# DINT-NSDI24/DINT

Measured on NVIDIA H100. Metric: committed txns/sec (lock_fasst), higher is better.
Workload: dtype u32

## Files before the change

### dint_b200/csrc/engine.cu

```cuda
#include <cmath>
#include <cstdio>
#include <cstdlib>
#include <cstring>
#include <string>
#include <chrono>
#include <vector>

#include "../../include/dint_b200.h"
#include "kernels.cuh"
#include "route.cuh"
#include "kv.cuh"
#include "clients.cuh"

using namespace dint;

static thread_local std::string g_last_error;
static int set_err(int code, const char* what, cudaError_t ce = cudaSuccess) {
  char buf[512];
  if (ce != cudaSuccess) snprintf(buf, sizeof buf, "%s: %s", what, cudaGetErrorString(ce));
  else snprintf(buf, sizeof buf, "%s", what);
  g_last_error = buf;
  return code;
}
#define CU(call)                                                              \
// ... 7 lines not shown
static const uint32_t kValSize[DINT_NUM_KINDS] = {0, 0, 0, 40, 40, 8};

enum { KT_CLASSIFY = 0, KT_LOGSCAN, KT_APPLY, KT_ORDERED, KT_LOAD, KT_NUM };
static const char* kKernelNames[KT_NUM] = {"k_classify", "k_log_scan", "k_apply", "k_ordered", "k_kv_load"};

struct EvPair { cudaEvent_t a, b; int which; };
constexpr int kHostBufs = 4;

struct dint_engine {
  int kind = 0;
  int device = 0;
  dint_cfg cfg{};
  uint32_t msg = 0;
  uint32_t chunk = 0;
  uint32_t max_tiles = 0;
  bool has_log = false;
  Ctx ctx{};
  std::vector<void*> allocs;
  cudaStream_t stream = nullptr, s_in = nullptr, s_out = nullptr;
  uint8_t* d_req[kHostBufs] = {nullptr};
  uint8_t* d_resp[kHostBufs] = {nullptr};
  cudaEvent_t ev_in[kHostBufs]{}, ev_comp[kHostBufs]{}, ev_out[kHostBufs]{};
  uint32_t host_chunk = 0;
  bool plain_launches = false;
  uint32_t host_min_slice = 0;
  bool host_ramp_up = true;
  unsigned long long* h_counters = nullptr;
  unsigned long long* h_kvcnt = nullptr;
  cudaEvent_t ev_kvcnt = nullptr;
  int coop_grid = 0;
  int sms = 0;
  int grid_classify = 0, grid_apply = 0;
  uint32_t smem_stage = 0;
  uint64_t total_groups = 0;
  uint32_t* d_flags[2] = {nullptr, nullptr};
  uint32_t* d_grp[2] = {nullptr, nullptr};
  uint64_t chunk_seq = 0;
  uint32_t prev_n = 0;
  bool ord_pending = false;
  uint8_t* ord_resp = nullptr;
  const uint8_t* ord_req = nullptr;
  uint32_t ord_tile0 = 0;
  uint32_t seg_tiles = 0;
  uint64_t seg_resp[kMaxShards]{};
  bool pad_ok = false;
  const uint32_t* skip = nullptr;
  uint32_t smem_classify = 0;
  uint32_t* d_nc = nullptr;
  uint32_t* d_route = nullptr;
  uint32_t route_tiles = 0;
  uint32_t* d_route2 = nullptr;
  uint32_t route_desc_tiles = 0, route_seq = 0;
  int grid_route = 0;
  uint8_t* hot_arena = nullptr;
  size_t hot_bytes = 0;
  bool use_window = false;
  cudaAccessPolicyWindow window{};
  dint_stats stats{};
  uint32_t profiling = 0;
  std::vector<EvPair> ev_pool;
  size_t ev_used = 0;
  double kt_ms[KT_NUM] = {0};
  uint64_t kt_n[KT_NUM] = {0};
  KvHost kv[kMaxTables];
};

template <typename T>
static int dalloc(dint_engine* e, T** p, size_t count, bool zero = true) {
// ... 24 lines not shown
    e->stats.kernel_launches++;
    if (!((e->profiling >> which) & 1u)) return;
    if (e->ev_used == e->ev_pool.size()) {
      if (e->ev_pool.size() >= 8192) { prof_flush(e); }
      else {
        EvPair np{}; cudaEventCreate(&np.a); cudaEventCreate(&np.b);
        e->ev_pool.push_back(np);
      }
    }
    p = &e->ev_pool[e->ev_used++];
    p->which = which;
    cudaEventRecord(p->a, s);
  }
  ~ProfScope() { if (p) cudaEventRecord(p->b, s); }
};

template <typename... Args>
static cudaError_t launch_ex(dint_engine* e, void (*kern)(Args...), int grid, int block, size_t smem, cudaStream_t s,
                             bool coop, Args... args) {
  cudaLaunchConfig_t cfg{};
  cfg.gridDim = dim3(grid < 1 ? 1 : grid);
  cfg.blockDim = dim3(block);
  cfg.dynamicSmemBytes = smem;
  cfg.stream = s;
  cudaLaunchAttribute at[3];
  int na = 0;
  if (coop) { at[na].id = cudaLaunchAttributeCooperative; at[na].val.cooperative = 1; na++; }
  if (e->use_window) { at[na].id = cudaLaunchAttributeAccessPolicyWindow; at[na].val.accessPolicyWindow = e->window; na++; }
  cfg.attrs = at;
  cfg.numAttrs = na;
  return cudaLaunchKernelEx(&cfg, kern, args...);
}

template <int KIND, bool HAS_LOG>
static int launch_chunk_t(dint_engine* e, const Ctx& c, cudaStream_t s) {
  {
    ProfScope ps(e, s, KT_CLASSIFY);
    int want = (int)c.n_tiles, clr = (int)((c.prev_n + 4 * kTile - 1) / (4 * kTile));
    if (clr > want) want = clr;
    int grid = (want < e->grid_classify && !c.ord_pending) ? want : e->grid_classify;
    if (c.n == 0 && e->sms > 0 && grid > 8 * e->sms) grid = 8 * e->sms;
    CU(launch_ex(e, k_classify<KIND, HAS_LOG>, grid, kTile, e->smem_classify, s, false, c));
  }
  if (c.n == 0) { CU(cudaGetLastError()); return DINT_OK; }
  if (HAS_LOG) {
    ProfScope ps(e, s, KT_LOGSCAN);
    k_log_scan<<<1, kThreads, 0, s>>>(c);
  }
  {
    ProfScope ps(e, s, KT_APPLY);
    int grid = (int)c.n_tiles < e->grid_apply ? (int)c.n_tiles : e->grid_apply;
    CU(launch_ex(e, k_apply<KIND, HAS_LOG>, grid, kTile, e->smem_stage, s, false, c));
  }
  if (KIND != K_LOG) {
    ProfScope ps(e, s, KT_ORDERED);
    Ctx f = c;
    f.nc_ord = c.nc_cur;
    f.ord_resp = c.resp;
    f.ord_req = c.req;
    f.ord_tile0 = c.tile0;
    f.coop_launch = e->plain_launches ? 0u : 1u;
    int g3 = e->coop_grid;
    if (e->plain_launches && e->sms > 0) {
      const int per = g3 / e->sms;
      g3 = (per > 1 ? per - 1 : 1) * e->sms;
    }
    CU(launch_ex(e, k_ordered<KIND>, g3, kThreads, 0, s, !e->plain_launches, f));
  }
// ... 2 lines not shown
}

static int launch_chunk(dint_engine* e, const Ctx& c, cudaStream_t s) {
  switch (e->kind) {
    case DINT_LOCK2PL: return launch_chunk_t<K_LOCK2PL, false>(e, c, s);
    case DINT_FASST: return launch_chunk_t<K_FASST, false>(e, c, s);
    case DINT_LOG: return launch_chunk_t<K_LOG, true>(e, c, s);
    case DINT_STORE: return launch_chunk_t<K_STORE, false>(e, c, s);
    case DINT_TATP: return launch_chunk_t<K_TATP, true>(e, c, s);
    case DINT_SMALLBANK: return launch_chunk_t<K_SMALLBANK, true>(e, c, s);
  }
  return DINT_EINVAL;
}

template <int KIND, bool HAS_LOG>
static int grids_for(dint_engine* e) {
  int per_sm = 0, sms = 0;
  CU(cudaDeviceGetAttribute(&sms, cudaDevAttrMultiProcessorCount, e->device));
  e->sms = sms;
  e->grid_route = 4 * sms;
  e->smem_stage = Stage<Wire<KIND>::MSG>::N * Stage<Wire<KIND>::MSG>::BYTES;
  if (e->smem_stage > 48 * 1024) {
    CU(cudaFuncSetAttribute(k_classify<KIND, HAS_LOG>, cudaFuncAttributeMaxDynamicSharedMemorySize, (int)e->smem_stage));
    CU(cudaFuncSetAttribute(k_apply<KIND, HAS_LOG>, cudaFuncAttributeMaxDynamicSharedMemorySize, (int)e->smem_stage));
  }
  e->smem_classify = e->smem_stage;
  if (KIND != K_LOG && (kTile / 32) * OrdSlice<KIND>::BYTES > e->smem_classify) e->smem_classify = (kTile / 32) * OrdSlice<KIND>::BYTES;
  CU(cudaOccupancyMaxActiveBlocksPerMultiprocessor(&per_sm, k_classify<KIND, HAS_LOG>, kTile, e->smem_classify));
  if (per_sm < 1) return set_err(DINT_EIO, "k_classify cannot be resident");
  e->grid_classify = per_sm * sms;
  CU(cudaOccupancyMaxActiveBlocksPerMultiprocessor(&per_sm, k_apply<KIND, HAS_LOG>, kTile, e->smem_stage));
  if (per_sm < 1) return set_err(DINT_EIO, "k_apply cannot be resident");
  e->grid_apply = per_sm * sms;
  if (KIND == K_LOG) { e->coop_grid = 1; return DINT_OK; }
  CU(cudaOccupancyMaxActiveBlocksPerMultiprocessor(&per_sm, k_ordered<KIND>, kThreads, 0));
  if (per_sm < 1) return set_err(DINT_EIO, "k_ordered cannot be resident");
  if (per_sm > 4) per_sm = 4;
  e->coop_grid = per_sm * sms;
  return DINT_OK;
}

static void fill_chunk_ctx(dint_engine* e, Ctx& c) {
  const int cur = (int)(e->chunk_seq & 1);
  c.grp = e->d_grp[cur];
  c.grp_prev = e->d_grp[cur ^ 1];
  c.flags = e->d_flags[cur];
  c.flags_prev = e->d_flags[cur ^ 1];
  c.prev_n = e->prev_n;
  c.nc_cur = e->d_nc + 4 * cur;
  c.nc_ord = e->d_nc + 4 * (cur ^ 1);
  c.ord_pending = e->ord_pending ? 1u : 0u;
  c.ord_resp = e->ord_resp;
  c.ord_req = e->ord_req;
  c.ord_tile0 = e->ord_tile0;
  c.seg_tiles = e->seg_tiles;
  c.pad_ok = e->pad_ok ? 1u : 0u;
  c.skip = e->skip;
  for (int i = 0; i < kMaxShards; i++) c.seg_resp[i] = e->seg_resp[i];
}

static int submit_chunk(dint_engine* e, const uint8_t* req, uint32_t n, uint8_t* resp, cudaStream_t s, uint32_t tile0 = 0) {
  Ctx c = e->ctx;
  c.n = n;
  c.n_tiles = (n + kTile - 1) / kTile;
  c.req = req;
  c.resp = resp;
  c.tile0 = tile0;
  fill_chunk_ctx(e, c);
  int rc = launch_chunk(e, c, s);
  if (rc) return rc;
  e->chunk_seq++;
  e->prev_n = n;
  e->ord_pending = e->kind != DINT_LOG;
  e->ord_resp = resp;
  e->ord_req = req;
  e->ord_tile0 = tile0;
  e->stats.chunks++;
  e->stats.requests += n;
  return DINT_OK;
}

static int flush_ordered(dint_engine* e, cudaStream_t s) {
  if (!e->ord_pending) return DINT_OK;
  Ctx c = e->ctx;
  c.n = 0;
  c.n_tiles = 0;
  c.req = nullptr;
  c.resp = nullptr;
  fill_chunk_ctx(e, c);
  c.prev_n = 0;
  int rc = launch_chunk(e, c, s);
  if (rc) return rc;
  e->ord_pending = false;
  return DINT_OK;
}

static int kv_maintain(dint_engine* e, cudaStream_t s) {
  if (e->ctx.n_tables == 0) return DINT_OK;
  if (!e->h_kvcnt) {
    CU(cudaHostAlloc((void**)&e->h_kvcnt, 2 * kMaxTables * sizeof(unsigned long long), cudaHostAllocDefault));
    memset(e->h_kvcnt, 0, 2 * kMaxTables * sizeof(unsigned long long));
    CU(cudaEventCreateWithFlags(&e->ev_kvcnt, cudaEventDisableTiming));
    return DINT_OK;
  }
  if (cudaEventQuery(e->ev_kvcnt) != cudaSuccess) { cudaGetLastError(); return DINT_OK; }
  for (uint32_t t = 0; t < e->ctx.n_tables; t++) {
// ... 211 lines not shown
  c.shard_id = cf.shard_id;
  c.shard_div = make_fastmod(cf.n_shards);
  c.slot_mod = make_fastmod(cf.lock_slots);
  c.ring_n = cf.log_ring ? cf.log_ring : 1;

  uint64_t groups = 0;
  auto local_groups = [&](uint64_t global) { return (global + cf.n_shards - 1) / cf.n_shards; };
  int rc;
  switch (e->kind) {
    case DINT_LOCK2PL:
      groups = local_groups(cf.lock_slots);
      if ((rc = dalloc(e, &c.cnt2, groups))) return rc;
      break;
    case DINT_FASST:
      groups = local_groups(cf.lock_slots);
      if ((rc = dalloc(e, &c.ver, groups))) return rc;
      break;
    case DINT_LOG:
      groups = 0;
      break;
    default:
      if ((rc = kv_create_tables(e->kind, cf, c, e->kv, &groups,
                                 [&](void** p, size_t bytes) -> int {
                                   uint8_t* q = nullptr;
                                   int r = dalloc(e, &q, bytes);
                                   *p = q;
                                   return r;
                                 })))
        return rc == DINT_EINVAL ? set_err(rc, "bad KV configuration") : rc;
      break;
  }
  e->total_groups = groups;
  if (groups >= 0xffffffffULL) return set_err(DINT_EINVAL, "too many groups");
  {
    uint32_t fl = 25;
    while (fl > 10 && (1ULL << (fl - 1)) >= groups * 2 + 2048) fl--;
    c.flags_mask = (1u << fl) - 1;
    const size_t set_bytes = (size_t)4 << (fl - 3);
    const size_t lock_bytes = (e->kind == DINT_FASST) ? (((groups + 31) / 32) * 4 + 255) / 256 * 256 : 0;
    e->hot_bytes = 2 * set_bytes + lock_bytes;
    if ((rc = dalloc(e, &e->hot_arena, e->hot_bytes))) return rc;
    e->d_flags[0] = (uint32_t*)e->hot_arena;
    e->d_flags[1] = (uint32_t*)(e->hot_arena + set_bytes);
    if (lock_bytes) c.lockbits = (uint32_t*)(e->hot_arena + 2 * set_bytes);
    int max_persist = 0, max_win = 0;
    cudaDeviceGetAttribute(&max_persist, cudaDevAttrMaxPersistingL2CacheSize, e->device);
    cudaDeviceGetAttribute(&max_win, cudaDevAttrMaxAccessPolicyWindowSize, e->device);
    if (max_persist > 0 && max_win > 0) {
      size_t want = e->hot_bytes < (size_t)max_persist ? e->hot_bytes : (size_t)max_persist;
      if (cudaDeviceSetLimit(cudaLimitPersistingL2CacheSize, want) == cudaSuccess) {
        e->window.base_ptr = e->hot_arena;
        e->window.num_bytes = e->hot_bytes < (size_t)max_win ? e->hot_bytes : (size_t)max_win;
        e->window.hitRatio = (float)((double)want / (double)e->window.num_bytes > 1.0 ? 1.0 : (double)want / (double)e->window.num_bytes);
        e->window.hitProp = cudaAccessPropertyPersisting;
        e->window.missProp = cudaAccessPropertyStreaming;
        e->use_window = true;
      } else cudaGetLastError();
    }
  }
  uint32_t bits = 1;
  while ((1ULL << bits) < groups) bits++;
  c.sort_passes = (bits + 7) / 8;

  if (e->has_log) {
    if ((rc = dalloc(e, &c.ring, (size_t)c.ring_n * kLogEntry[e->kind]))) return rc;
  }
  const uint32_t ch = e->chunk;
  e->max_tiles = (ch + kTile - 1) / kTile;
  for (int i = 0; i < 2; i++)
    if ((rc = dalloc(e, &e->d_grp[i], ch))) return rc;
  if ((rc = dalloc(e, &c.clist, (size_t)e->max_tiles * kTile))) return rc;
  if ((rc = dalloc(e, &c.ccnt, e->max_tiles))) return rc;
  if ((rc = dalloc(e, &c.cprefix, e->max_tiles + 1))) return rc;
  if ((rc = dalloc(e, &e->d_nc, 8))) return rc;
  {
    uint32_t lg = 0;
    while (((uint64_t)kBucketFill << lg) < ch) lg++;
    c.bucket_log2 = lg;
    if ((rc = dalloc(e, &c.buckets, ((size_t)1 << lg) * kBucketCap, false))) return rc;
    if ((rc = dalloc(e, &c.bcnt, (size_t)1 << lg))) return rc;
  }
  if ((rc = dalloc(e, &c.sortA, ch))) return rc;
  if ((rc = dalloc(e, &c.sortB, ch))) return rc;
  if ((rc = dalloc(e, &c.ghist, (size_t)256 * ((ch + kSortTile - 1) / kSortTile)))) return rc;
  if ((rc = dalloc(e, &c.rowtot, 256))) return rc;
  if ((rc = dalloc(e, &c.log_tilecnt, e->max_tiles))) return rc;
  if ((rc = dalloc(e, &c.log_tilebase, e->max_tiles))) return rc;
  if ((rc = dalloc(e, &c.log_total, 2))) return rc;
  if ((rc = dalloc(e, &c.counters, 4))) return rc;
  if ((rc = dalloc(e, &c.gbar, 4))) return rc;

  switch (e->kind) {
    case DINT_LOCK2PL: rc = grids_for<K_LOCK2PL, false>(e); break;
    case DINT_FASST: rc = grids_for<K_FASST, false>(e); break;
    case DINT_LOG: rc = grids_for<K_LOG, true>(e); break;
    case DINT_STORE: rc = grids_for<K_STORE, false>(e); break;
    case DINT_TATP: rc = grids_for<K_TATP, true>(e); break;
    default: rc = grids_for<K_SMALLBANK, true>(e); break;
  }
  if (rc) return rc;
  int coop = 0;
  CU(cudaDeviceGetAttribute(&coop, cudaDevAttrCooperativeLaunch, e->device));
  if (!coop) return set_err(DINT_ENODEV, "device lacks cooperative launch");
  CU(cudaStreamSynchronize(e->stream));
  return DINT_OK;
}

int dint_create(int kind, const dint_cfg* cfg, int device, dint_engine** out) {
  if (!out || kind < 0 || kind >= DINT_NUM_KINDS) return set_err(DINT_EINVAL, "bad kind/out");
  *out = nullptr;
  int ndev = 0;
  cudaError_t ce = cudaGetDeviceCount(&ndev);
  if (ce != cudaSuccess || ndev == 0) {
    cudaGetLastError();
    return set_err(DINT_ENODEV, "no CUDA device: dint_b200 has no CPU fallback");
  }
  if (device < 0 || device >= ndev) return set_err(DINT_EINVAL, "bad device ordinal");
  dint_engine* e = new dint_engine();
  e->kind = kind;
  e->device = device;
  if (cfg) e->cfg = *cfg; else dint_default_cfg(kind, &e->cfg);
  dint_cfg& cf = e->cfg;
  if (cf.n_shards == 0) cf.n_shards = 1;
  if (cf.shard_id >= cf.n_shards || cf.lock_slots == 0) { delete e; return set_err(DINT_EINVAL, "bad shard/lock_slots"); }
  if (cf.chunk == 0) cf.chunk = 1u << 20;
  e->chunk = (cf.chunk + kTile - 1) / kTile * kTile;
  {
    const uint32_t want = 1u << 18;
    e->host_chunk = want < e->chunk ? want : e->chunk;
    e->host_min_slice = 131072u;
    e->host_ramp_up = true;
  }
  e->msg = kMsgSize[kind];
// ... 167 lines not shown
  unsigned long long before = e->stats.errors;
  if ((rc = pull_counters(e))) return rc;
  return e->stats.errors != before ? DINT_EPROTO : DINT_OK;
}

int dint_submit_device(dint_engine* e, const void* req_dev, uint64_t n, void* resp_dev, void* cuda_stream) {
  if (!e || (n && (!req_dev || !resp_dev))) return set_err(DINT_EINVAL, "null argument");
  if (((uintptr_t)req_dev | (uintptr_t)resp_dev) & 15) return set_err(DINT_EINVAL, "device buffers must be 16-byte aligned");
  CU(cudaSetDevice(e->device));
  cudaStream_t s = (cudaStream_t)cuda_stream;
  return run_device(e, (const uint8_t*)req_dev, n, (uint8_t*)resp_dev, s);
}

int dint_submit(dint_engine* e, const void* req, uint64_t n, void* resp) {
  if (!e || (n && (!req || !resp))) return set_err(DINT_EINVAL, "null argument");
  CU(cudaSetDevice(e->device));
  const uint32_t hchunk = e->host_chunk;
  if (!e->d_req[0]) {
    for (int i = 0; i < kHostBufs; i++) {
      int rc;
      if ((rc = dalloc(e, &e->d_req[i], (size_t)hchunk * e->msg + 16, false))) return rc;
      if ((rc = dalloc(e, &e->d_resp[i], (size_t)hchunk * e->msg + 16, false))) return rc;
    }
  }
  static const bool trace = getenv("DINT_HOST_TRACE") != nullptr;
  const auto t_begin = std::chrono::steady_clock::now();
  CU(cudaDeviceSynchronize());
  { int rc = kv_maintain(e, e->stream); if (rc) return rc; }
  const uint8_t* rq = (const uint8_t*)req;
  uint8_t* rs = (uint8_t*)resp;
  unsigned long long err_before = e->stats.errors;
  uint64_t k = 0;
  uint64_t prev_off = 0, prev_bytes = 0;
  auto copy_out_prev = [&](uint64_t kk) -> int {
    int pb = (int)((kk - 1) % kHostBufs);
    CU(cudaEventRecord(e->ev_comp[pb], e->stream));
    CU(cudaStreamWaitEvent(e->s_out, e->ev_comp[pb], 0));
    CU(cudaMemcpyAsync(rs + prev_off, e->d_resp[pb], prev_bytes, cudaMemcpyDeviceToHost, e->s_out));
    CU(cudaEventRecord(e->ev_out[pb], e->s_out));
    return DINT_OK;
  };
  HostSlices sched(n, e->host_min_slice, hchunk, e->host_ramp_up);
  uint64_t off = 0;
  for (uint64_t cn; (cn = sched.next()) != 0; k++) {
    int b = (int)(k % kHostBufs);
    size_t bytes = (size_t)cn * e->msg;
    if (k >= (uint64_t)kHostBufs) CU(cudaStreamWaitEvent(e->s_in, e->ev_comp[b], 0));
    CU(cudaMemcpyAsync(e->d_req[b], rq + off * e->msg, bytes, cudaMemcpyHostToDevice, e->s_in));
    CU(cudaEventRecord(e->ev_in[b], e->s_in));
    CU(cudaStreamWaitEvent(e->stream, e->ev_in[b], 0));
    if (k >= (uint64_t)kHostBufs) CU(cudaStreamWaitEvent(e->stream, e->ev_out[b], 0));
    int rc = submit_chunk(e, e->d_req[b], (uint32_t)cn, e->d_resp[b], e->stream);
    if (rc) return rc;
    if (k >= 1 && (rc = copy_out_prev(k))) return rc;
    prev_off = off * e->msg;
    prev_bytes = bytes;
    e->stats.h2d_bytes += bytes;
    e->stats.d2h_bytes += bytes;
    off += cn;
  }
  {
    int rc = flush_ordered(e, e->stream);
    if (rc) return rc;
    if (k >= 1 && (rc = copy_out_prev(k))) return rc;
  }
  if (!e->h_counters) CU(cudaHostAlloc((void**)&e->h_counters, 4 * sizeof(unsigned long long), cudaHostAllocDefault));
  CU(cudaMemcpyAsync(e->h_counters, e->ctx.counters, 4 * sizeof(unsigned long long), cudaMemcpyDeviceToHost, e->stream));
  { int rc2 = kv_publish_counts(e, e->stream); if (rc2) return rc2; }
  const auto t_enq = std::chrono::steady_clock::now();
  CU(cudaStreamSynchronize(e->s_out));
  CU(cudaStreamSynchronize(e->stream));
  int rc = prof_flush(e);
  if (rc) return rc;
  if (trace) {
    const auto t_end = std::chrono::steady_clock::now();
    fprintf(stderr, "[dint_submit] n=%llu slices=%llu enqueue=%.1f us total=%.1f us\n", (unsigned long long)n, (unsigned long long)k,
            std::chrono::duration<double, std::micro>(t_enq - t_begin).count(),
            std::chrono::duration<double, std::micro>(t_end - t_begin).count());
  }
  e->stats.errors = e->h_counters[0];
  e->stats.conflicted = e->h_counters[1];
  e->stats.max_run = e->h_counters[2];
  return e->stats.errors != err_before ? DINT_EPROTO : DINT_OK;
}

struct dint_snapshot {
  dint_engine* e = nullptr;
  std::vector<std::pair<void*, size_t>> live;
  std::vector<void*> copy;
  uint64_t kv_cap[kMaxTables]{};
};
static void snapshot_regions(dint_engine* e, std::vector<std::pair<void*, size_t>>& r) {
  const Ctx& c = e->ctx;
  const uint64_t g = e->total_groups;
  if (e->kind == DINT_LOCK2PL || e->kind == DINT_SMALLBANK) r.push_back({c.cnt2, g * sizeof(uint2)});
  if (e->kind == DINT_FASST) { r.push_back({c.ver, g * sizeof(uint32_t)}); r.push_back({c.lockbits, ((g + 31) / 32) * 4}); }
  if (e->kind == DINT_TATP) r.push_back({c.lockbits, ((g + 31) / 32) * 4});
// ... 475 lines not shown
  if (c->flags) cudaFree(c->flags);
  if (c->side) cudaStreamDestroy(c->side);
  if (c->ret) cudaStreamDestroy(c->ret);
  if (c->s_in) cudaStreamDestroy(c->s_in);
  if (c->s_out) cudaStreamDestroy(c->s_out);
  c->e->plain_launches = false;
  delete c;
}

int dint_shard_flags(dint_shard_ctx* c, uint32_t out[2]) {
  if (!c || !out) return DINT_EINVAL;
  CU(cudaSetDevice(c->e->device));
  CU(cudaDeviceSynchronize());
  CU(cudaMemcpy(out, c->flags, 2 * sizeof(uint32_t), cudaMemcpyDeviceToHost));
  CU(cudaMemset(c->flags, 0, 2 * sizeof(uint32_t)));
  return DINT_OK;
}

int dint_shard_recover(dint_shard_ctx* c, uint32_t k_last, uint32_t* first_unserved) {
  if (!c || !first_unserved) return DINT_EINVAL;
  dint_engine* e = c->e;
  CU(cudaSetDevice(e->device));
  CU(cudaDeviceSynchronize());
  uint32_t bad = 0;
  CU(cudaMemcpy(&bad, c->flags + 2, sizeof bad, cudaMemcpyDeviceToHost));
  *first_unserved = 0xffffffffu;
  if (!bad) return DINT_OK;
  const uint32_t first_epoch = c->epoch - k_last + 1;
  *first_unserved = bad >= first_epoch ? bad - first_epoch : 0;
  CU(cudaMemset(c->flags, 0, 4 * sizeof(uint32_t)));
  e->ord_pending = false;
  e->prev_n = 0;
  CU(cudaMemset(e->d_nc, 0, 8 * sizeof(uint32_t)));
  CU(cudaMemset(e->d_flags[0], 0, (size_t)((char*)e->d_flags[1] - (char*)e->d_flags[0]) * 2));
  CU(cudaDeviceSynchronize());
  return DINT_OK;
}

int dint_shard_submit_many(dint_shard_ctx* c, uint32_t k, const void* const* req_dev, const uint8_t* const* dst_dev, uint64_t n,
                           void* const* out_dev, void* cuda_stream) {
  if (!c || !req_dev || !out_dev || n == 0 || n > c->max_n) return set_err(DINT_EINVAL, "bad argument");
  if (k == 0) return DINT_OK;
  std::vector<std::vector<ShardBatch>> b(1, std::vector<ShardBatch>(k));
  for (uint32_t j = 0; j < k; j++) b[0][j] = ShardBatch{req_dev[j], dst_dev ? dst_dev[j] : nullptr, out_dev[j], n};
  cudaStream_t main = (cudaStream_t)cuda_stream;
  return shard_run(&c, 1, k, b, &main);
}

}

extern "C" {

int dint_shard_submit_many_v(dint_shard_ctx* c, uint32_t k, const void* const* req_dev, const uint8_t* const* dst_dev, const uint64_t* n,
                             const uint32_t* cap, void* const* out_dev, void* cuda_stream) {
  if (!c || !req_dev || !out_dev || !n) return set_err(DINT_EINVAL, "bad argument");
  if (k == 0) return DINT_OK;
  std::vector<std::vector<ShardBatch>> b(1, std::vector<ShardBatch>(k));
  for (uint32_t j = 0; j < k; j++) {
    const uint32_t cj = cap ? cap[j] : 0;
    if (n[j] > c->max_n || cj > c->cap || cj % kTile != 0) return set_err(DINT_EINVAL, "batch size / slab capacity (a multiple of 128, <= the capacity of dint_shard_create)");
    b[0][j] = ShardBatch{req_dev[j], dst_dev ? dst_dev[j] : nullptr, out_dev[j], n[j], cj};
  }
  cudaStream_t main = (cudaStream_t)cuda_stream;
  return shard_run(&c, 1, k, b, &main);
}

int dint_shard_submit_host(dint_shard_ctx* c, uint32_t k, const void* const* req_host, const uint8_t* const* dst_host, uint64_t n,
// ... 284 lines not shown
```

### dint_b200/csrc/kernels.cuh

```cuda
#pragma once
#include <cooperative_groups.h>
#include "engine.cuh"

namespace dint {
namespace cg = cooperative_groups;

DINT_D uint32_t lane_id() { return threadIdx.x & 31; }
DINT_D uint32_t warp_id() { return threadIdx.x >> 5; }

DINT_D uint32_t tile_rank(bool flag, uint32_t* scratch, uint32_t& total) {
  uint32_t bal = __ballot_sync(0xffffffffu, flag);
  uint32_t in_warp = __popc(bal & ((1u << lane_id()) - 1u));
  if (lane_id() == 0) scratch[warp_id()] = __popc(bal);
  __syncthreads();
  uint32_t off = 0, tot = 0;
#pragma unroll
  for (int w = 0; w < kTile / 32; w++) {
    uint32_t v = scratch[w];
    if (w < (int)warp_id()) off += v;
    tot += v;
  }
  __syncthreads();
  total = tot;
  return off + in_warp;
// ... 4 lines not shown
  const uint32_t lt = (1u << lane_id()) - 1u;
  if (lane_id() == 0) scratch[warp_id()] = __popc(ba) | (__popc(bb) << 16);
  __syncthreads();
  uint32_t off = 0, tot = 0;
#pragma unroll
  for (int w = 0; w < kTile / 32; w++) {
    uint32_t v = scratch[w];
    if (w < (int)warp_id()) off += v;
    tot += v;
  }
  ra = (off & 0xffffu) + __popc(ba & lt);
  rb = (off >> 16) + __popc(bb & lt);
  ta = tot & 0xffffu;
  tb = tot >> 16;
}

DINT_D uint32_t bucket_of(uint32_t g, uint32_t log2p) { return log2p ? (g * 0x9E3779B1u) >> (32 - log2p) : 0; }

template <int MSG> struct Stage {
  static constexpr uint32_t BYTES = ((kTile * MSG + 16 + 127) / 128) * 128;
  static constexpr uint32_t N = (BYTES > 8192) ? 2 : kStages;
};

struct TileIter {
  uint32_t n_my;
  DINT_D uint32_t tile(uint32_t i) const { return blockIdx.x + i * gridDim.x; }
  DINT_D bool has(uint32_t i) const { return i < n_my; }
};
DINT_D TileIter tile_iter(uint32_t n_tiles) {
  TileIter it;
  it.n_my = blockIdx.x < n_tiles ? (n_tiles - blockIdx.x + gridDim.x - 1) / gridDim.x : 0;
  return it;
}
template <int MSG>
DINT_D void issue_tile_load(const Ctx& c, uint8_t* smem, uint64_t* full, const TileIter& it, uint32_t i) {
  const uint32_t t = it.tile(i), first = t * kTile;
  const uint32_t cnt = min((uint32_t)kTile, c.n - first);
  const uint32_t body = (cnt * MSG) & ~15u;
  const uint32_t buf = i % Stage<MSG>::N;
  if (body) {
    mbar_expect_tx(&full[buf], body);
    tma_load_1d(smem + buf * Stage<MSG>::BYTES, c.req + (size_t)first * MSG, body, &full[buf]);
  }
}
template <int MSG>
DINT_D uint8_t* acquire_tile(const Ctx& c, uint8_t* smem, uint64_t* full, const TileIter& it, uint32_t i,
                             uint32_t& first, uint32_t& cnt) {
  const uint32_t t = it.tile(i);
  first = t * kTile;
  cnt = min((uint32_t)kTile, c.n - first);
  const uint32_t bytes = cnt * MSG, body = bytes & ~15u;
  uint8_t* tile = smem + (i % Stage<MSG>::N) * Stage<MSG>::BYTES;
  if (body) mbar_wait(&full[i % Stage<MSG>::N], (i / Stage<MSG>::N) & 1u);
  if (body != bytes) {
    const uint8_t* src = c.req + (size_t)first * MSG;
    for (uint32_t b = body + threadIdx.x; b < bytes; b += blockDim.x) tile[b] = src[b];
    __syncthreads();
  }
  return tile;
}

template <int KIND>
DINT_D uint32_t route_owner_of(const Ctx& c, const uint8_t* rec) {
  using W = Wire<KIND>;
  const TypeInfo ti = type_info<KIND>(rec);
  if (ti.invalid || !ti.mask) return c.shard_id;
  uint32_t gglobal = 0;
  if constexpr (KIND == K_LOCK2PL || KIND == K_FASST) gglobal = fast_mod(fasthash64_u32(ld_u32_unaligned(rec + W::KEY)), c.slot_mod);
  else if constexpr (KIND == K_STORE) gglobal = fast_mod(fasthash64_u64(ld_u64_unaligned(rec + W::KEY)), c.tbl[0].lock_mod);
  else if constexpr (KIND == K_TATP || KIND == K_SMALLBANK) gglobal = fast_mod(fasthash64_u64(ld_u64_unaligned(rec + W::KEY)), c.tbl[rec[W::TABLE]].lock_mod);
  else return c.shard_id;
  return gglobal - (uint32_t)fast_div(gglobal, c.shard_div) * c.n_shards;
}
template <int KIND>
__global__ void __launch_bounds__(kThreads) k_route_owner(const Ctx c, const uint8_t* req, uint32_t n, uint8_t* owner) {
  const uint32_t i = blockIdx.x * kThreads + threadIdx.x;
  if (i < n) owner[i] = (uint8_t)route_owner_of<KIND>(c, req + (size_t)i * Wire<KIND>::MSG);
}

constexpr int kMaxShards = 8;
__global__ void __launch_bounds__(kThreads) k_exact_count(const uint8_t* owner, uint32_t n, uint32_t world, uint32_t* tilecnt) {
  __shared__ uint32_t cnt[kMaxShards];
  if (threadIdx.x < kMaxShards) cnt[threadIdx.x] = 0;
  __syncthreads();
  const uint32_t i = blockIdx.x * kThreads + threadIdx.x;
  const uint32_t o = i < n ? owner[i] : 0xffu;
// ... 60 lines not shown
    __threadfence_system();
    volatile uint32_t* flag = (volatile uint32_t*)sig.p[threadIdx.x] + me;
    asm volatile("st.release.sys.global.u32 [%0], %1;" ::"l"(flag), "r"(epoch) : "memory");
  }
}
constexpr uint32_t kSigOverflow = 0x80000000u;
__global__ void k_p2p_wait(const uint32_t* my_sig, uint32_t world, uint32_t epoch, uint32_t* timeout, uint32_t* bad) {
  if (threadIdx.x < world) {
    const long long t0 = clock64();
    uint32_t v;
    do {
      asm volatile("ld.acquire.sys.global.u32 %0, [%1];" : "=r"(v) : "l"(my_sig + threadIdx.x) : "memory");
      if (clock64() - t0 > 8000000000LL) { atomicExch(timeout, 1u); break; }
    } while ((int32_t)((v & ~kSigOverflow) - epoch) < 0);
    if (bad && (v & kSigOverflow) && (v & ~kSigOverflow) == epoch) atomicCAS(bad, 0u, epoch);
  }
  __syncthreads();
  __threadfence_system();
}

template <int MSG>
__global__ void __launch_bounds__(kThreads) k_exact_unpermute(const uint8_t* sorted, const uint32_t* perm, uint32_t n, uint8_t* out) {
  const uint32_t pos = blockIdx.x * kThreads + threadIdx.x;
  if (pos >= n) return;
  const uint32_t idx = perm[pos];
  if (idx == 0xffffffffu) return;
  copy_record<MSG>(out + (size_t)idx * MSG, sorted + (size_t)pos * MSG);
}

template <int KIND> struct OrdSlice {
  static constexpr uint32_t BYTES = kBucketCap * (FastReplay<KIND>::ok ? (8 + 8 + 4) : 8);
};
template <int KIND> DINT_D void ordered_buckets(const Ctx& c, uint8_t* scratch);

template <int KIND, bool HAS_LOG>
__global__ void __launch_bounds__(kTile) k_classify(const Ctx c) {
  using W = Wire<KIND>;
  constexpr uint32_t NS = Stage<W::MSG>::N;
  extern __shared__ __align__(128) uint8_t smem[];
  __shared__ uint64_t full[kStages];
  __shared__ uint32_t scratch[kTile / 32];
  if (c.skip && __ldcg(c.skip)) return;
  if (threadIdx.x == 0) {
    for (int s = 0; s < kStages; s++) mbar_init(&full[s], 1);
    if (blockIdx.x == 0) { c.nc_cur[0] = 0; c.nc_cur[1] = 0; c.nc_ord[2] = 0; }
  }
  __syncthreads();
  const bool do_ord = c.ord_pending && c.nc_ord[0] != 0 && c.nc_ord[1] == 0;
  const bool ord_first = (blockIdx.x & 1u) != 0;
  if (do_ord && ord_first) {
    ordered_buckets<KIND>(c, smem);
    __syncthreads();
  }
  const TileIter it = tile_iter(c.n_tiles);
  if (threadIdx.x == 0)
    for (uint32_t i = 0; i < NS && i < it.n_my; i++) issue_tile_load<W::MSG>(c, smem, full, it, i);

  for (uint32_t i = blockIdx.x * kTile + threadIdx.x; i < c.prev_n; i += 4 * gridDim.x * kTile) {
    uint32_t g[4];
#pragma unroll
    for (int u = 0; u < 4; u++) {
      const uint32_t j = i + u * gridDim.x * kTile;
      g[u] = j < c.prev_n ? __ldcg(&c.grp_prev[j]) : kNoGroup;
    }
#pragma unroll
    for (int u = 0; u < 4; u++)
      if (g[u] != kNoGroup) c.flags_prev[flag_word(c, g[u])] = 0;
  }

  uint32_t pend_old = 0, pend_test = 0, pend_sh = 0;
  uint32_t* pend_w = nullptr;
  bool saw_writer = false;
  for (uint32_t i = 0; it.has(i); i++) {
    if (threadIdx.x == 0 && i && i + NS - 1 < it.n_my) issue_tile_load<W::MSG>(c, smem, full, it, i + NS - 1);
    uint32_t first, cnt;
    const uint8_t* tile = acquire_tile<W::MSG>(c, smem, full, it, i, first, cnt);
    const bool valid = threadIdx.x < cnt;
    bool is_log = false;
    uint32_t new_old = 0, new_test = 0, new_sh = 0;
    uint32_t* new_w = nullptr;
    if (valid) {
      const uint8_t* rec = tile + threadIdx.x * W::MSG;
      TypeInfo ti = (c.pad_ok && rec[W::TYPE] == kPadType) ? TypeInfo{0, false, false} : type_info<KIND>(rec);
      uint32_t g = kNoGroup;
      if (!ti.invalid && ti.mask) {
        g = key_info<KIND>(c, rec).grp;
        if (g != kNoGroup) {
          uint32_t* w = &c.flags[flag_word(c, g)];
          const uint32_t sh = flag_shift(g);
          if (ti.mask == C_RA) {
            atomicOr(w, F_R << sh);
          } else {
            const uint32_t bits = ((ti.mask & C_RA) ? F_R : 0u) | ((ti.mask & C_WA) ? F_WA : 0u) | ((ti.mask & C_WL) ? F_WL : 0u);
            saw_writer = true;
            new_old = atomicOr(w, bits << sh);
            new_test = ((ti.mask & C_WA) ? F_WA : 0u) | ((ti.mask & C_WL) ? F_WL : 0u);
            new_w = w;
            new_sh = sh;
          }
        }
      }
      c.grp[first + threadIdx.x] = g;
      is_log = !ti.invalid && ti.is_log;
    }
    if (pend_w && ((pend_old >> pend_sh) & pend_test)) atomicOr(pend_w, F_W2 << pend_sh);
    pend_old = new_old; pend_test = new_test; pend_sh = new_sh; pend_w = new_w;
    if (HAS_LOG) {
      uint32_t total;
      (void)tile_rank(is_log, scratch, total);
      if (threadIdx.x == 0) c.log_tilecnt[it.tile(i)] = total;
    } else {
      __syncthreads();
    }
  }
  if (pend_w && ((pend_old >> pend_sh) & pend_test)) atomicOr(pend_w, F_W2 << pend_sh);
  if (__syncthreads_or(saw_writer ? 1 : 0) && threadIdx.x == 0) atomicOr(&c.nc_cur[2], 1u);
  if (do_ord && !ord_first) {
    __syncthreads();
    ordered_buckets<KIND>(c, smem);
  }
}

__global__ void __launch_bounds__(kThreads) k_log_scan(const Ctx c) {
  if (c.skip && __ldcg(c.skip)) return;
  __shared__ unsigned long long carry;
  __shared__ uint32_t wsum[kThreads / 32];
  if (threadIdx.x == 0) carry = c.log_total[0];
  __syncthreads();
  for (uint32_t base = 0; base < c.n_tiles; base += kThreads) {
// ... 44 lines not shown
  for (uint32_t i = 0; it.has(i); i++) {
    uint32_t* scratch = scratch2[i & 1];
    uint32_t g_k1 = kNoGroup;
    if (kGrpFromK1) {
      const uint32_t idx = it.tile(i) * kTile + threadIdx.x;
      if (idx < c.n) g_k1 = __ldcg(&c.grp[idx]);
    }
    if (threadIdx.x == 0 && i && i + NS - 1 < it.n_my) {
      asm volatile("cp.async.bulk.wait_group.read 0;" ::: "memory");
      issue_tile_load<W::MSG>(c, smem, full, it, i + NS - 1);
    }
    uint32_t first, cnt;
    uint8_t* tile = acquire_tile<W::MSG>(c, smem, full, it, i, first, cnt);
    const uint32_t t = it.tile(i);
    const bool valid = threadIdx.x < cnt;
    uint8_t* rec = tile + threadIdx.x * W::MSG;
    TypeInfo ti{0, false, false};
    KeyInfo ki{0, 0, kNoGroup};
    Pre<KIND> pf;
    bool listed = false;
    const bool pad = valid && c.pad_ok && rec[W::TYPE] == kPadType;
    if (valid && !pad) {
      ti = type_info<KIND>(rec);
      if (!ti.invalid && ti.mask) {
        if (kGrpFromK1) ki.grp = g_k1; else ki = key_info<KIND>(c, rec);
        if (ki.grp == kNoGroup) ti.invalid = true;
      }
    }
    {
      const bool active = valid && !ti.invalid && ti.mask;
      pf = prefetch_coop<KIND>(c, rec, ki, ti, active);
      if (active && chunk_has_writer) {
        const uint32_t f = (__ldcg(&c.flags[flag_word(c, ki.grp)]) >> flag_shift(ki.grp)) & 15u;
        listed = ((ti.mask & C_RA) && (f & F_WA)) || ((ti.mask & C_WA) && (f & (F_R | F_W2))) ||
                 ((ti.mask & C_WL) && (f & F_W2));
      }
    }
    unsigned long long log_ord = 0;
    bool log_keep = false;
    {
      const bool lg = HAS_LOG && valid && !ti.invalid && ti.is_log;
      uint32_t r_list, r_log, n_list, n_log;
      tile_rank2(listed, lg, scratch, r_list, r_log, n_list, n_log);
      if (lg) {
        log_ord = c.log_tilebase[t] + r_log;
        log_keep = log_ord + c.ring_n >= c.log_total[1];
      }
      if (listed) {
        const uint32_t idx = first + threadIdx.x;
        c.clist[(size_t)t * kTile + r_list] = idx;
        const uint32_t b = bucket_of(ki.grp, c.bucket_log2);
        const uint32_t pos = atomicAdd(&c.bcnt[b], 1u);
        if (pos < kBucketCap) c.buckets[(size_t)b * kBucketCap + pos] = ((uint64_t)ki.grp << 32) | idx;
        else atomicAdd(&c.nc_cur[1], 1u);
      }
      if (threadIdx.x == 0) {
        c.ccnt[t] = n_list;
        if (n_list) atomicAdd(&c.nc_cur[0], n_list);
      }
    }
    if (valid && !pad) {
      if (ti.invalid) mark_invalid<KIND>(c, rec);
      else if (!listed) apply_one<KIND>(c, rec, ki, pf, log_ord, log_keep);
    }
    const uint32_t bytes = cnt * W::MSG, body = bytes & ~15u;
    uint8_t* gdst = c.seg_tiles ? seg_tile_ptr<W::MSG>(c, c.tile0 + t) : c.resp + (size_t)first * W::MSG;
    fence_proxy_async_smem();
    __syncthreads();
    for (uint32_t b = body + threadIdx.x; b < bytes; b += blockDim.x) gdst[b] = tile[b];
    if (threadIdx.x == 0) {
      if (body) tma_store_1d(gdst, tile, body);
      asm volatile("cp.async.bulk.commit_group;" ::: "memory");
    }
  }
  if (threadIdx.x == 0) asm volatile("cp.async.bulk.wait_group 0;" ::: "memory");
}

constexpr int kSortItems = 8;
constexpr int kSortTile = kThreads * kSortItems;

template <int KIND>
DINT_D void replay_run(const Ctx& c, const uint64_t* sorted, uint32_t p, uint32_t nc) {
  using W = Wire<KIND>;
  const uint32_t g = (uint32_t)(sorted[p] >> 32);
  uint32_t len = 0;
  for (uint32_t q = p; q < nc; q++) {
    uint64_t e = sorted[q];
    if ((uint32_t)(e >> 32) != g) break;
    __align__(4) uint8_t rec[(W::MSG + 3) / 4 * 4];
    copy_record<W::MSG>(rec, c.ord_req + (size_t)(uint32_t)e * W::MSG);
    const TypeInfo ti = type_info<KIND>(rec);
    const KeyInfo ki = key_info<KIND>(c, rec);
    const Pre<KIND> pf = prefetch<KIND>(c, rec, ki, ti);
    apply_one<KIND>(c, rec, ki, pf, 0, false);
    copy_record<W::MSG>(ord_out_ptr<W::MSG>(c, (uint32_t)e), rec);
    len++;
  }
  if (len > 1) atomicMax(&c.counters[2], (unsigned long long)len);
}

template <int KIND>
DINT_D void ordered_buckets(const Ctx& c, uint8_t* scratch) {
    uint64_t* wkeys = (uint64_t*)(scratch + (size_t)warp_id() * OrdSlice<KIND>::BYTES);
    uint64_t* wres = wkeys + kBucketCap;
    uint32_t* wops = (uint32_t*)(wkeys + 2 * kBucketCap);
    const uint32_t lane = lane_id();
    const uint32_t warps_per_cta = blockDim.x / 32;
    const uint32_t n_warps = gridDim.x * warps_per_cta;
// ... 440 lines not shown
```

Before: 280.5 million.

## Fuse classify, apply and ordered replay into one cooperative kernel for FASST/2PL

Result: faster. 380.0 million (median of 6 runs) (+35.5%).

```diff
diff --git a/dint_b200/csrc/engine.cu b/dint_b200/csrc/engine.cu
--- a/dint_b200/csrc/engine.cu
+++ b/dint_b200/csrc/engine.cu
@@ -63,8 +63,11 @@
   int sms = 0;
   int grid_classify = 0, grid_apply = 0;
   uint32_t smem_stage = 0;
+  bool fused_kind = false;
+  int grid_fused = 0;
   uint64_t total_groups = 0;
   uint32_t* d_flags[2] = {nullptr, nullptr};
+  size_t flag_set_bytes = 0;
   uint32_t* d_grp[2] = {nullptr, nullptr};
   uint64_t chunk_seq = 0;
   uint32_t prev_n = 0;
@@ -155,8 +158,32 @@
   return cudaLaunchKernelEx(&cfg, kern, args...);
 }
 
+static bool fused_path(const dint_engine* e) { return e->fused_kind && !e->plain_launches; }
+
 template <int KIND, bool HAS_LOG>
 static int launch_chunk_t(dint_engine* e, const Ctx& c, cudaStream_t s) {
+  if constexpr (KIND == K_FASST || KIND == K_LOCK2PL) {
+    if (fused_path(e)) {
+      Ctx f = c;
+      f.flags = e->d_flags[0];
+      f.nc_ord = c.nc_cur;
+      f.ord_resp = c.resp;
+      f.ord_req = c.req;
+      f.ord_tile0 = c.tile0;
+      f.coop_launch = 1;
+      {
+        ProfScope ps(e, s, KT_APPLY);
+        const int grid = (int)c.n_tiles < e->grid_fused ? (int)c.n_tiles : e->grid_fused;
+        CU(launch_ex(e, k_fused<KIND>, grid, kTile, Fused<KIND>::SMEM, s, true, f));
+      }
+      {
+        ProfScope ps(e, s, KT_ORDERED);
+        CU(launch_ex(e, k_ordered<KIND>, e->coop_grid, kThreads, 0, s, true, f));
+      }
+      CU(cudaGetLastError());
+      return DINT_OK;
+    }
+  }
   {
     ProfScope ps(e, s, KT_CLASSIFY);
     int want = (int)c.n_tiles, clr = (int)((c.prev_n + 4 * kTile - 1) / (4 * kTile));
@@ -225,6 +252,12 @@
   CU(cudaOccupancyMaxActiveBlocksPerMultiprocessor(&per_sm, k_apply<KIND, HAS_LOG>, kTile, e->smem_stage));
   if (per_sm < 1) return set_err(DINT_EIO, "k_apply cannot be resident");
   e->grid_apply = per_sm * sms;
+  if constexpr (KIND == K_FASST || KIND == K_LOCK2PL) {
+    CU(cudaOccupancyMaxActiveBlocksPerMultiprocessor(&per_sm, k_fused<KIND>, kTile, Fused<KIND>::SMEM));
+    if (per_sm < 1) return set_err(DINT_EIO, "k_fused cannot be resident");
+    e->fused_kind = true;
+    e->grid_fused = per_sm * sms;
+  }
   if (KIND == K_LOG) { e->coop_grid = 1; return DINT_OK; }
   CU(cudaOccupancyMaxActiveBlocksPerMultiprocessor(&per_sm, k_ordered<KIND>, kThreads, 0));
   if (per_sm < 1) return set_err(DINT_EIO, "k_ordered cannot be resident");
@@ -259,12 +292,17 @@
   c.req = req;
   c.resp = resp;
   c.tile0 = tile0;
+  const bool fused = fused_path(e);
+  if (fused && e->prev_n) {
+    CU(cudaMemsetAsync(e->d_flags[(e->chunk_seq - 1) & 1], 0, e->flag_set_bytes, s));
+    e->prev_n = 0;
+  }
   fill_chunk_ctx(e, c);
   int rc = launch_chunk(e, c, s);
   if (rc) return rc;
   e->chunk_seq++;
-  e->prev_n = n;
-  e->ord_pending = e->kind != DINT_LOG;
+  e->prev_n = fused ? 0 : n;
+  e->ord_pending = !fused && e->kind != DINT_LOG;
   e->ord_resp = resp;
   e->ord_req = req;
   e->ord_tile0 = tile0;
@@ -542,17 +580,37 @@
   }
   e->total_groups = groups;
   if (groups >= 0xffffffffULL) return set_err(DINT_EINVAL, "too many groups");
+  switch (e->kind) {
+    case DINT_LOCK2PL: rc = grids_for<K_LOCK2PL, false>(e); break;
+    case DINT_FASST: rc = grids_for<K_FASST, false>(e); break;
+    case DINT_LOG: rc = grids_for<K_LOG, true>(e); break;
+    case DINT_STORE: rc = grids_for<K_STORE, false>(e); break;
+    case DINT_TATP: rc = grids_for<K_TATP, true>(e); break;
+    default: rc = grids_for<K_SMALLBANK, true>(e); break;
+  }
+  if (rc) return rc;
+  if (e->fused_kind) {
+    const uint64_t cap = (uint64_t)e->grid_fused * kFuseTiles * kTile;
+    if (e->chunk > cap) e->chunk = (uint32_t)cap;
+    if (e->host_chunk > e->chunk) e->host_chunk = e->chunk;
+  }
   {
     uint32_t fl = 25;
     while (fl > 10 && (1ULL << (fl - 1)) >= groups * 2 + 2048) fl--;
     c.flags_mask = (1u << fl) - 1;
     const size_t set_bytes = (size_t)4 << (fl - 3);
+    e->flag_set_bytes = set_bytes;
     const size_t lock_bytes = (e->kind == DINT_FASST) ? (((groups + 31) / 32) * 4 + 255) / 256 * 256 : 0;
-    e->hot_bytes = 2 * set_bytes + lock_bytes;
+    const size_t hot_sets = e->fused_kind ? 1 : 2;
+    e->hot_bytes = hot_sets * set_bytes + lock_bytes;
     if ((rc = dalloc(e, &e->hot_arena, e->hot_bytes))) return rc;
     e->d_flags[0] = (uint32_t*)e->hot_arena;
-    e->d_flags[1] = (uint32_t*)(e->hot_arena + set_bytes);
-    if (lock_bytes) c.lockbits = (uint32_t*)(e->hot_arena + 2 * set_bytes);
+    if (e->fused_kind) {
+      if ((rc = dalloc(e, &e->d_flags[1], set_bytes / 4))) return rc;
+    } else {
+      e->d_flags[1] = (uint32_t*)(e->hot_arena + set_bytes);
+    }
+    if (lock_bytes) c.lockbits = (uint32_t*)(e->hot_arena + hot_sets * set_bytes);
     int max_persist = 0, max_win = 0;
     cudaDeviceGetAttribute(&max_persist, cudaDevAttrMaxPersistingL2CacheSize, e->device);
     cudaDeviceGetAttribute(&max_win, cudaDevAttrMaxAccessPolicyWindowSize, e->device);
@@ -600,15 +658,6 @@
   if ((rc = dalloc(e, &c.counters, 4))) return rc;
   if ((rc = dalloc(e, &c.gbar, 4))) return rc;
 
-  switch (e->kind) {
-    case DINT_LOCK2PL: rc = grids_for<K_LOCK2PL, false>(e); break;
-    case DINT_FASST: rc = grids_for<K_FASST, false>(e); break;
-    case DINT_LOG: rc = grids_for<K_LOG, true>(e); break;
-    case DINT_STORE: rc = grids_for<K_STORE, false>(e); break;
-    case DINT_TATP: rc = grids_for<K_TATP, true>(e); break;
-    default: rc = grids_for<K_SMALLBANK, true>(e); break;
-  }
-  if (rc) return rc;
   int coop = 0;
   CU(cudaDeviceGetAttribute(&coop, cudaDevAttrCooperativeLaunch, e->device));
   if (!coop) return set_err(DINT_ENODEV, "device lacks cooperative launch");
@@ -842,11 +891,12 @@
   unsigned long long err_before = e->stats.errors;
   uint64_t k = 0;
   uint64_t prev_off = 0, prev_bytes = 0;
-  auto copy_out_prev = [&](uint64_t kk) -> int {
-    int pb = (int)((kk - 1) % kHostBufs);
+  bool pending = false;
+  auto copy_out = [&](uint64_t kk, uint64_t at, uint64_t nbytes) -> int {
+    int pb = (int)(kk % kHostBufs);
     CU(cudaEventRecord(e->ev_comp[pb], e->stream));
     CU(cudaStreamWaitEvent(e->s_out, e->ev_comp[pb], 0));
-    CU(cudaMemcpyAsync(rs + prev_off, e->d_resp[pb], prev_bytes, cudaMemcpyDeviceToHost, e->s_out));
+    CU(cudaMemcpyAsync(rs + at, e->d_resp[pb], nbytes, cudaMemcpyDeviceToHost, e->s_out));
     CU(cudaEventRecord(e->ev_out[pb], e->s_out));
     return DINT_OK;
   };
@@ -862,7 +912,9 @@
     if (k >= (uint64_t)kHostBufs) CU(cudaStreamWaitEvent(e->stream, e->ev_out[b], 0));
     int rc = submit_chunk(e, e->d_req[b], (uint32_t)cn, e->d_resp[b], e->stream);
     if (rc) return rc;
-    if (k >= 1 && (rc = copy_out_prev(k))) return rc;
+    if (pending && (rc = copy_out(k - 1, prev_off, prev_bytes))) return rc;
+    pending = e->ord_pending;
+    if (!pending && (rc = copy_out(k, off * e->msg, bytes))) return rc;
     prev_off = off * e->msg;
     prev_bytes = bytes;
     e->stats.h2d_bytes += bytes;
@@ -872,7 +924,7 @@
   {
     int rc = flush_ordered(e, e->stream);
     if (rc) return rc;
-    if (k >= 1 && (rc = copy_out_prev(k))) return rc;
+    if (pending && (rc = copy_out(k - 1, prev_off, prev_bytes))) return rc;
   }
   if (!e->h_counters) CU(cudaHostAlloc((void**)&e->h_counters, 4 * sizeof(unsigned long long), cudaHostAllocDefault));
   CU(cudaMemcpyAsync(e->h_counters, e->ctx.counters, 4 * sizeof(unsigned long long), cudaMemcpyDeviceToHost, e->stream));
@@ -1414,7 +1466,8 @@
   e->ord_pending = false;
   e->prev_n = 0;
   CU(cudaMemset(e->d_nc, 0, 8 * sizeof(uint32_t)));
-  CU(cudaMemset(e->d_flags[0], 0, (size_t)((char*)e->d_flags[1] - (char*)e->d_flags[0]) * 2));
+  CU(cudaMemset(e->d_flags[0], 0, e->flag_set_bytes));
+  CU(cudaMemset(e->d_flags[1], 0, e->flag_set_bytes));
   CU(cudaDeviceSynchronize());
   return DINT_OK;
 }
diff --git a/dint_b200/csrc/kernels.cuh b/dint_b200/csrc/kernels.cuh
--- a/dint_b200/csrc/kernels.cuh
+++ b/dint_b200/csrc/kernels.cuh
@@ -60,26 +60,26 @@
   it.n_my = blockIdx.x < n_tiles ? (n_tiles - blockIdx.x + gridDim.x - 1) / gridDim.x : 0;
   return it;
 }
-template <int MSG>
+template <int MSG, uint32_t NB = Stage<MSG>::N, uint32_t BUF = Stage<MSG>::BYTES>
 DINT_D void issue_tile_load(const Ctx& c, uint8_t* smem, uint64_t* full, const TileIter& it, uint32_t i) {
   const uint32_t t = it.tile(i), first = t * kTile;
   const uint32_t cnt = min((uint32_t)kTile, c.n - first);
   const uint32_t body = (cnt * MSG) & ~15u;
-  const uint32_t buf = i % Stage<MSG>::N;
+  const uint32_t buf = i % NB;
   if (body) {
     mbar_expect_tx(&full[buf], body);
-    tma_load_1d(smem + buf * Stage<MSG>::BYTES, c.req + (size_t)first * MSG, body, &full[buf]);
-  }
-}
-template <int MSG>
+    tma_load_1d(smem + buf * BUF, c.req + (size_t)first * MSG, body, &full[buf]);
+  }
+}
+template <int MSG, uint32_t NB = Stage<MSG>::N, uint32_t BUF = Stage<MSG>::BYTES>
 DINT_D uint8_t* acquire_tile(const Ctx& c, uint8_t* smem, uint64_t* full, const TileIter& it, uint32_t i,
                              uint32_t& first, uint32_t& cnt) {
   const uint32_t t = it.tile(i);
   first = t * kTile;
   cnt = min((uint32_t)kTile, c.n - first);
   const uint32_t bytes = cnt * MSG, body = bytes & ~15u;
-  uint8_t* tile = smem + (i % Stage<MSG>::N) * Stage<MSG>::BYTES;
-  if (body) mbar_wait(&full[i % Stage<MSG>::N], (i / Stage<MSG>::N) & 1u);
+  uint8_t* tile = smem + (i % NB) * BUF;
+  if (body) mbar_wait(&full[i % NB], (i / NB) & 1u);
   if (body != bytes) {
     const uint8_t* src = c.req + (size_t)first * MSG;
     for (uint32_t b = body + threadIdx.x; b < bytes; b += blockDim.x) tile[b] = src[b];
@@ -206,6 +206,28 @@
   static constexpr uint32_t BYTES = kBucketCap * (FastReplay<KIND>::ok ? (8 + 8 + 4) : 8);
 };
 template <int KIND> DINT_D void ordered_buckets(const Ctx& c, uint8_t* scratch);
+
+DINT_D uint32_t flag_bits(uint32_t mask) {
+  return ((mask & C_RA) ? F_R : 0u) | ((mask & C_WA) ? F_WA : 0u) | ((mask & C_WL) ? F_WL : 0u);
+}
+DINT_D uint32_t writer_bits(uint32_t mask) { return ((mask & C_WA) ? F_WA : 0u) | ((mask & C_WL) ? F_WL : 0u); }
+DINT_D bool conflicts(uint32_t mask, uint32_t f) {
+  return ((mask & C_RA) && (f & F_WA)) || ((mask & C_WA) && (f & (F_R | F_W2))) || ((mask & C_WL) && (f & F_W2));
+}
+DINT_D void list_request(const Ctx& c, uint32_t t, uint32_t first, bool listed, uint32_t grp, uint32_t r_list, uint32_t n_list) {
+  if (listed) {
+    const uint32_t idx = first + threadIdx.x;
+    c.clist[(size_t)t * kTile + r_list] = idx;
+    const uint32_t b = bucket_of(grp, c.bucket_log2);
+    const uint32_t pos = atomicAdd(&c.bcnt[b], 1u);
+    if (pos < kBucketCap) c.buckets[(size_t)b * kBucketCap + pos] = ((uint64_t)grp << 32) | idx;
+    else atomicAdd(&c.nc_cur[1], 1u);
+  }
+  if (threadIdx.x == 0) {
+    c.ccnt[t] = n_list;
+    if (n_list) atomicAdd(&c.nc_cur[0], n_list);
+  }
+}
 
 template <int KIND, bool HAS_LOG>
 __global__ void __launch_bounds__(kTile) k_classify(const Ctx c) {
@@ -265,10 +287,9 @@
           if (ti.mask == C_RA) {
             atomicOr(w, F_R << sh);
           } else {
-            const uint32_t bits = ((ti.mask & C_RA) ? F_R : 0u) | ((ti.mask & C_WA) ? F_WA : 0u) | ((ti.mask & C_WL) ? F_WL : 0u);
             saw_writer = true;
-            new_old = atomicOr(w, bits << sh);
-            new_test = ((ti.mask & C_WA) ? F_WA : 0u) | ((ti.mask & C_WL) ? F_WL : 0u);
+            new_old = atomicOr(w, flag_bits(ti.mask) << sh);
+            new_test = writer_bits(ti.mask);
             new_w = w;
             new_sh = sh;
           }
@@ -379,8 +400,7 @@
       pf = prefetch_coop<KIND>(c, rec, ki, ti, active);
       if (active && chunk_has_writer) {
         const uint32_t f = (__ldcg(&c.flags[flag_word(c, ki.grp)]) >> flag_shift(ki.grp)) & 15u;
-        listed = ((ti.mask & C_RA) && (f & F_WA)) || ((ti.mask & C_WA) && (f & (F_R | F_W2))) ||
-                 ((ti.mask & C_WL) && (f & F_W2));
+        listed = conflicts(ti.mask, f);
       }
     }
     unsigned long long log_ord = 0;
@@ -393,18 +413,7 @@
         log_ord = c.log_tilebase[t] + r_log;
         log_keep = log_ord + c.ring_n >= c.log_total[1];
       }
-      if (listed) {
-        const uint32_t idx = first + threadIdx.x;
-        c.clist[(size_t)t * kTile + r_list] = idx;
-        const uint32_t b = bucket_of(ki.grp, c.bucket_log2);
-        const uint32_t pos = atomicAdd(&c.bcnt[b], 1u);
-        if (pos < kBucketCap) c.buckets[(size_t)b * kBucketCap + pos] = ((uint64_t)ki.grp << 32) | idx;
-        else atomicAdd(&c.nc_cur[1], 1u);
-      }
-      if (threadIdx.x == 0) {
-        c.ccnt[t] = n_list;
-        if (n_list) atomicAdd(&c.nc_cur[0], n_list);
-      }
+      list_request(c, t, first, listed, ki.grp, r_list, n_list);
     }
     if (valid && !pad) {
       if (ti.invalid) mark_invalid<KIND>(c, rec);
@@ -421,6 +430,134 @@
     }
   }
   if (threadIdx.x == 0) asm volatile("cp.async.bulk.wait_group 0;" ::: "memory");
+}
+
+constexpr int kFuseTiles = 8;
+template <int KIND> struct Fused {
+  static constexpr uint32_t TILE = (kTile * Wire<KIND>::MSG + 15) / 16 * 16;
+  static constexpr uint32_t TILES = kFuseTiles * TILE;
+  static constexpr uint32_t REPLAY = (kTile / 32) * OrdSlice<KIND>::BYTES;
+  static constexpr uint32_t GRP = TILES > REPLAY ? TILES : REPLAY;
+  static constexpr uint32_t SMEM = GRP + kFuseTiles * kTile * 4;
+};
+
+template <int KIND>
+__global__ void __launch_bounds__(kTile, 8) k_fused(const Ctx c) {
+  using W = Wire<KIND>;
+  using F = Fused<KIND>;
+  extern __shared__ __align__(128) uint8_t smem[];
+  __shared__ uint64_t full[kFuseTiles];
+  __shared__ uint32_t scratch2[2][kTile / 32];
+  uint32_t* s_grp = (uint32_t*)(smem + F::GRP);
+  cg::grid_group grid = cg::this_grid();
+  const TileIter it = tile_iter(c.n_tiles);
+  const uint32_t tid = threadIdx.x;
+  if (tid == 0) {
+    for (int s = 0; s < kFuseTiles; s++) mbar_init(&full[s], 1);
+    if (blockIdx.x == 0) { c.nc_cur[0] = 0; c.nc_cur[1] = 0; }
+  }
+  __syncthreads();
+  if (tid == 0)
+    for (uint32_t i = 0; i < it.n_my; i++) issue_tile_load<W::MSG, kFuseTiles, F::TILE>(c, smem, full, it, i);
+
+  Pre<KIND> pf[kFuseTiles];
+  uint32_t old[kFuseTiles];
+  uint32_t wtest = 0;
+  bool saw_writer = false;
+#pragma unroll
+  for (int i = 0; i < kFuseTiles; i++) {
+    old[i] = 0;
+    pf[i] = Pre<KIND>{};
+    if (!it.has(i)) continue;
+    uint32_t first, cnt;
+    const uint8_t* tile = acquire_tile<W::MSG, kFuseTiles, F::TILE>(c, smem, full, it, i, first, cnt);
+    uint32_t g = kNoGroup;
+    if (tid < cnt) {
+      const uint8_t* rec = tile + tid * W::MSG;
+      const TypeInfo ti = type_info<KIND>(rec);
+      if (!ti.invalid) {
+        const KeyInfo ki = key_info<KIND>(c, rec);
+        g = ki.grp;
+        if (g != kNoGroup) {
+          uint32_t* w = &c.flags[flag_word(c, g)];
+          const uint32_t sh = flag_shift(g);
+          if (ti.mask == C_RA) {
+            atomicOr(w, F_R << sh);
+          } else {
+            saw_writer = true;
+            old[i] = atomicOr(w, flag_bits(ti.mask) << sh);
+            wtest |= writer_bits(ti.mask) << (4 * i);
+          }
+          pf[i] = prefetch<KIND>(c, rec, ki, ti);
+        }
+      }
+      c.grp[first + tid] = g;
+    }
+    s_grp[i * kTile + tid] = g;
+  }
+#pragma unroll
+  for (int i = 0; i < kFuseTiles; i++) {
+    const uint32_t test = (wtest >> (4 * i)) & 15u;
+    if (test) {
+      const uint32_t g = s_grp[i * kTile + tid];
+      if ((old[i] >> flag_shift(g)) & test) atomicOr(&c.flags[flag_word(c, g)], F_W2 << flag_shift(g));
+    }
+  }
+  if (__syncthreads_or(saw_writer ? 1 : 0) && tid == 0) atomicOr(&c.nc_cur[2], 1u);
+  grid.sync();
+
+  const bool chunk_has_writer = __ldcg(&c.nc_cur[2]) != 0;
+  uint32_t fl[kFuseTiles];
+#pragma unroll
+  for (int i = 0; i < kFuseTiles; i++) {
+    fl[i] = 0;
+    const uint32_t g = it.has(i) ? s_grp[i * kTile + tid] : kNoGroup;
+    if (chunk_has_writer && g != kNoGroup) fl[i] = (__ldcg(&c.flags[flag_word(c, g)]) >> flag_shift(g)) & 15u;
+  }
+#pragma unroll
+  for (int i = 0; i < kFuseTiles; i++) {
+    if (!it.has(i)) continue;
+    const uint32_t t = it.tile(i), first = t * kTile, cnt = min((uint32_t)kTile, c.n - first);
+    uint8_t* rec = smem + i * F::TILE + tid * W::MSG;
+    const bool valid = tid < cnt;
+    const uint32_t g = s_grp[i * kTile + tid];
+    const TypeInfo ti = valid ? type_info<KIND>(rec) : TypeInfo{0, true, false};
+    const bool bad = ti.invalid || g == kNoGroup;
+    const bool listed = valid && !bad && conflicts(ti.mask, fl[i]);
+    uint32_t r_list, r_unused, n_list, n_unused;
+    tile_rank2(listed, false, scratch2[i & 1], r_list, r_unused, n_list, n_unused);
+    list_request(c, t, first, listed, g, r_list, n_list);
+    if (valid) {
+      if (bad) mark_invalid<KIND>(c, rec);
+      else if (!listed) apply_one<KIND>(c, rec, KeyInfo{0, 0, g}, pf[i], 0, false);
+    }
+  }
+  fence_proxy_async_smem();
+  __syncthreads();
+  if (tid == 0) {
+    for (uint32_t i = 0; i < it.n_my; i++) {
+      const uint32_t first = it.tile(i) * kTile, body = (min((uint32_t)kTile, c.n - first) * W::MSG) & ~15u;
+      if (body) tma_store_1d(c.resp + (size_t)first * W::MSG, smem + i * F::TILE, body);
+    }
+    asm volatile("cp.async.bulk.commit_group;" ::: "memory");
+  }
+  if (it.has(0) && it.tile(it.n_my - 1) == c.n_tiles - 1) {
+    const uint32_t i = it.n_my - 1, first = it.tile(i) * kTile, bytes = (c.n - first) * W::MSG;
+    for (uint32_t b = (bytes & ~15u) + tid; b < bytes; b += blockDim.x) c.resp[(size_t)first * W::MSG + b] = smem[i * F::TILE + b];
+  }
+  if (tid == 0) {
+    asm volatile("cp.async.bulk.wait_group 0;" ::: "memory");
+    asm volatile("fence.proxy.async.global;" ::: "memory");
+  }
+  grid.sync();
+
+#pragma unroll
+  for (int i = 0; i < kFuseTiles; i++) {
+    const uint32_t g = it.has(i) ? s_grp[i * kTile + tid] : kNoGroup;
+    if (g != kNoGroup) c.flags[flag_word(c, g)] = 0;
+  }
+  if (blockIdx.x == 0 && tid == 0) c.nc_cur[2] = 0;
+  if (__ldcg(&c.nc_ord[0]) != 0 && __ldcg(&c.nc_ord[1]) == 0) ordered_buckets<KIND>(c, smem);
 }
 
 constexpr int kSortItems = 8;
```
